# amolchanov86/gym_art

Hardware: AMD Instinct MI355X
Metric: env-steps/sec (whole node) at N=2^20 Hummingbird; achieved HBM GB/s (higher is better)
Workload: dtype f64

## Files before the change

gym_art_amd/csrc/gaq.hip:

```cpp
#include "gaq_host.hpp"

#define GAQ_X(FEAT) extern template __global__ GAQ_STEP_SIG(FEAT)
GAQ_STEP_ALL(GAQ_X)
#undef GAQ_X
#define GAQ_X(FEAT) extern template __global__ GAQ_ROLL_SIG(FEAT)
GAQ_ROLL_ALL(GAQ_X)
#undef GAQ_X

namespace {

using namespace gaqk;

__global__ __launch_bounds__(kBlock) void episode_kernel(int64_t n, const float* __restrict__ reward,
                                                          const uint8_t* __restrict__ done, float* __restrict__ ep_ret,
                                                          uint32_t* __restrict__ ep_len, double* __restrict__ acc) {
  const int64_t i = (int64_t)blockIdx.x * kBlock + threadIdx.x;
  float ret = 0.0f; uint32_t len = 0; bool fin = false;
  if (i < n) {
    ret = ep_ret[i] + reward[i];
    len = ep_len[i] + 1u;
    fin = done[i] != 0;
    ep_ret[i] = fin ? 0.0f : ret;
    ep_len[i] = fin ? 0u : len;
  }
// ... 141 lines not shown
      float* row = reinterpret_cast<float*>(rows) + lane * D;
      if (alias && !hi_out) {
#pragma unroll
        for (int k = 0; k < 18; ++k) row[k] = hi18[k];
      } else {
        const float* sz = p.sense_in;
        const int64_t n = p.n;
        double t2w = 0.0, t2t = 0.0;
        if (cfg.obs_flags & (gaq::OBS_APPEND_T2W | gaq::OBS_APPEND_T2T)) {
          double th[4], tq0 = um.torque_max[0], im = um.inv_mass;
#pragma unroll
          for (int j = 0; j < 4; ++j) th[j] = um.thrust_max[j];
          if (p.par) {
#pragma unroll
            for (int j = 0; j < 4; ++j) th[j] = t.ld64(p.par, kPar, PP_THRUST_MAX + j);
            tq0 = t.ld64(p.par, kPar, PP_TORQUE_MAX); im = t.ld64(p.par, kPar, PP_INV_MASS);
          }
          t2w = (((th[0] + th[1]) + th[2]) + th[3]) * im / 9.81; t2t = tq0 / th[0];
        }
        gaq::pack_obs<double, gaq::F_GENERIC | gaq::F_DIAG>(s, cfg, acc, hist, [&](int k, float v, int) { row[k] = v; },
                                            cfg.env_offset + (uint64_t)i, cfg.step_index, 1, WaveSwarm{lane, cfg.swarm.agents},
                                            [&](int c, int slot, int j) { return sz ? sz[((int64_t)(c * 12 + slot) * 3 + j) * n + i] : 0.0f; }, t2w, t2t);
        if (cfg.gyro_bias && (!do_reset || mask == nullptr || mask[i])) {
#pragma unroll
          for (int j = 0; j < 3; ++j) t.st32(p.gyro, j, s.gyro_bias[j]);
        }
      }
    }
  }
  if (obs) {
    wave_lds_fence();
    flush_obs(obs, p.n, D, tile, rows, lane);
  }
}

__global__ __launch_bounds__(kBlock) void export_kernel(DevPtrs p, int alias, double* __restrict__ out, float* __restrict__ aux_out = nullptr) {
  const int64_t i = (int64_t)blockIdx.x * kBlock + threadIdx.x;
  if (i >= p.n) return;
  if (aux_out) {
    for (int k = 0; k < gaq::AUX_WORDS; ++k) aux_out[i * gaq::AUX_WORDS + k] = p.aux[i * gaq::AUX_WORDS + k];
  }
  const int64_t n = p.n;
  const int64_t tile = i / kTile;
  const int lane = (int)(i % kTile);
  auto grp = [&](const float* a, int plane) { return (double)a[tile * (4 * kTile) + plane * kTile + lane]; };
  for (int k = 0; k < 3; ++k) out[(34 + k) * n + i] = grp(p.goal, k);
  if (alias) {
    for (int k = 0; k < 18; ++k)
      out[(int64_t)k * n + i] = lo_decode(alias, p.obs_in, p.lo, i, k) + (k < 3 ? grp(p.goal, k) : 0.0);
  } else {
    for (int k = 0; k < kCorePlanes; ++k) out[(int64_t)k * n + i] = p.core[tile * (kCorePlanes * kTile) + k * kTile + lane];
  }
  for (int j = 0; j < 4; ++j) {
    out[(18 + j) * n + i] = p.lag[tile * (kLagPlanes * kTile) + j * kTile + lane];
    out[(22 + j) * n + i] = grp(p.cmds, j);
    out[(26 + j) * n + i] = grp(p.ou, j);
    out[(30 + j) * n + i] = grp(p.actp, j);
  }
  const uint32_t c = p.ctr[i];
  out[37 * n + i] = (double)(c & 0xFFFFu);
  out[38 * n + i] = (double)(c >> 16);
  for (int k = 0; k < 3; ++k) out[(39 + k) * n + i] = grp(p.gyro, k);
}

thread_local std::string g_err;

int svd_period_of(double dt) {
  double t = 0.0; int k = 0;
  while (!(t > 0.5)) { t += dt; ++k; if (k > 1000000) break; }
  return k;
}

}

int fail(int code, const std::string& msg) { g_err = msg; return code; }
int env_override(const char* name) { const char* v = getenv(name); return v ? (v[0] == '1' ? 1 : 0) : -1; }
LaunchRecord& launch_record() { static LaunchRecord r; return r; }

namespace {

Overrides read_overrides() {
  return {env_override("GAQ_FORCE_GENERIC") == 1, env_override("GAQ_NO_AUXP") == 1, env_override("GAQ_PREDRAW"), env_override("GAQ_NT")};
}

struct Layout { bool alias, pack, shadow, fp32; };
struct Selection { uint32_t variant; bool generic; int lds_per_wave; };
struct ParamFlags { bool lag, drag; };
struct Plan { Layout layout; Selection sel; };

bool step_instantiated(uint32_t f) {
  switch (f) {
#define GAQ_X(FEAT) case (FEAT):
    GAQ_STEP_ALL(GAQ_X)
#undef GAQ_X
      return true;
    default: return false;
  }
}
bool roll_instantiated(uint32_t f) {
  switch (f) {
#define GAQ_X(FEAT) case (FEAT):
    GAQ_ROLL_ALL(GAQ_X)
#undef GAQ_X
      return true;
    default: return false;
  }
}

const void* step_kernel_ptr(uint32_t f) {
  switch (f) {
#define GAQ_X(FEAT) case (FEAT): return (const void*)&step_kernel<(FEAT)>;
    GAQ_STEP_ALL(GAQ_X)
#undef GAQ_X
    default: return nullptr;
  }
}
uint32_t rollout_variant_of(uint32_t variant, const Layout& L, bool generic) {
  const uint32_t base = variant & ~(gaq::F_PREDRAW | gaq::F_NT | gaq::F_ROWS | gaq::F_CTR);
  if (!L.alias || L.pack || generic || (variant & gaq::F_MELL)) return 0xFFFFFFFFu;
  if ((base >= 16u && base <= 23u) || (variant >= 48u && variant <= 55u)) return base;
  return 0xFFFFFFFFu;
}

uint32_t rows_twin_of(uint32_t variant) { return step_instantiated(variant | gaq::F_ROWS) ? (variant | gaq::F_ROWS) : 0xFFFFFFFFu; }
uint32_t ctr_twin_of(uint32_t variant) { return step_instantiated(variant | gaq::F_CTR) ? (variant | gaq::F_CTR) : 0xFFFFFFFFu; }

int observation_dim(const gaq_config* cfg) {
  int D = (cfg->obs_flags & GAQ_OBS_QUAT) ? 13 : 18;
  if (cfg->obs_flags & GAQ_OBS_APPEND_T2W) D += 1;
  if (cfg->obs_flags & GAQ_OBS_APPEND_T2T) D += 1;
  if (cfg->obs_flags & GAQ_OBS_APPEND_H) D += 1;
  if (cfg->obs_flags & GAQ_OBS_APPEND_ACC) D += 3;
  if (cfg->obs_flags & GAQ_OBS_APPEND_ACT) D += 4;
  if (cfg->swarm.agents > 1) D += 6 * (cfg->swarm.agents - 1);
  return D;
}

int fill_step_cfg(const gaq_config* cfg, StepCfg& sc, int& obs_dim) {
  if (cfg->struct_size != sizeof(gaq_config) || cfg->abi_version != GAQ_ABI_VERSION)
    return fail(GAQ_ERR_INVALID, "gaq_config size/version mismatch (header vs library)");
  if (cfg->num_envs <= 0) return fail(GAQ_ERR_INVALID, "num_envs must be positive");
  if (cfg->num_envs > (int64_t)1 << 27) return fail(GAQ_ERR_INVALID, "num_envs above 2^27 per handle is not supported");
  if (!(cfg->sim_freq > 0) || cfg->sim_steps <= 0) return fail(GAQ_ERR_INVALID, "sim_freq and sim_steps must be positive");
  if (cfg->sim_steps > 64)
    return fail(GAQ_ERR_INVALID, "sim_steps above 64 is not supported (random-stream ids of the sub-steps)");
  if (cfg->ep_len < 0 || cfg->ep_len >= 0xFFFF) return fail(GAQ_ERR_INVALID, "ep_len must be in [0, 65534]");
  if (cfg->control < 0 || cfg->control > 2) return fail(GAQ_ERR_INVALID, "unknown control mode");
  if (cfg->noise < 0 || cfg->noise > 2) return fail(GAQ_ERR_INVALID, "unknown noise mode");
  if (cfg->reward_mode < 0 || cfg->reward_mode > 1) return fail(GAQ_ERR_INVALID, "unknown reward mode");
  if (cfg->obs_flags & ~127) return fail(GAQ_ERR_INVALID, "unknown obs flags");
  if ((cfg->obs_flags & GAQ_OBS_QUAT) && cfg->swarm.agents > 1) return fail(GAQ_ERR_INVALID, "the quaternion observation is not available for swarms");
  if (cfg->swarm.agents > 1) {
    const int a = cfg->swarm.agents;
    if (a > 16 || (a & (a - 1)) != 0) return fail(GAQ_ERR_INVALID, "swarm.agents must be a power of two <= 16");
    if (cfg->num_envs % a != 0 || cfg->env_id_offset % a != 0)
      return fail(GAQ_ERR_INVALID, "num_envs and env_id_offset must be multiples of swarm.agents (whole worlds per handle)");
    if (!(cfg->swarm.prox_dist > 0.0f) || !(cfg->swarm.collision_dist >= 0.0f) || !(cfg->swarm.goal_radius >= 0.0f))
      return fail(GAQ_ERR_INVALID, "swarm distances must be positive");
  }
  const double dt = 1.0 / cfg->sim_freq;
  const int period = svd_period_of(dt);
  if (period >= 0xFFFF) return fail(GAQ_ERR_INVALID, "sim_freq too high for the 16-bit SVD counter");
  if (cfg->sim_freq < 50.0) return fail(GAQ_ERR_INVALID, "sim_freq below 50 Hz is outside the rotation series' range");
  const int D = observation_dim(cfg);
  obs_dim = D;
  std::memset(&sc, 0, sizeof(sc));
// ... 429 lines not shown
  if (e->stage_bytes > ((size_t)1 << 20)) return GAQ_OK;
  const bool zc = env_override("GAQ_ZERO_COPY") != 0;
  HIP_TRY(hipHostMalloc((void**)&e->stage_pin, e->stage_bytes, zc ? hipHostMallocMapped : hipHostMallocDefault));
  if (zc) e->stage_map = device_view(e->stage_pin);
  return GAQ_OK;
}

struct Transport {
  char* io;
  char* home;
  bool copy_in;
  bool own_obs;
};
Transport transport_of(const gaq_env* e) {
  const bool mapped = e->stage_map != nullptr;
  const bool own_obs = e->alias && !e->pack && !(mapped && e->shadow);
  return {mapped ? e->stage_map : e->stage_dev, e->stage_pin, !mapped, own_obs};
}

}

int sync_handle(gaq_env* e) {
  HIP_TRY(hipStreamSynchronize(e->stream));
  if (e->user_stream_used) HIP_TRY(hipStreamSynchronize(e->user_stream));
  return GAQ_OK;
}

int check_overrun(gaq_env* e) {
  if (!e->d.rz_overrun) return GAQ_OK;
  uint32_t o = 0;
  HIP_TRY(hipMemcpy(&o, e->d.rz_overrun, sizeof(uint32_t), hipMemcpyDeviceToHost));
  if (o) return fail(GAQ_ERR_STATE, "internal: an env was re-randomised before its staged parameter planes were refilled");
  return GAQ_OK;
}

extern "C" {

int gaq_abi_version(void) { return GAQ_ABI_VERSION; }
const char* gaq_last_error(void) { return g_err.c_str(); }

int gaq_num_devices(void) {
  int n = 0;
  if (hipGetDeviceCount(&n) != hipSuccess) return 0;
  return n;
}

int gaq_create(const gaq_config* cfg, gaq_env** out) {
  if (!cfg || !out) return fail(GAQ_ERR_INVALID, "null argument");
  StepCfg sc0;
  int D = 18;
  if (int rc = fill_step_cfg(cfg, sc0, D)) return rc;
  if (!cfg->per_env_params && check_model(cfg->model) != GAQ_OK) return GAQ_ERR_INVALID;
  int ndev = gaq_num_devices();
  if (ndev <= 0) return fail(GAQ_ERR_DEVICE, "no HIP device visible: libgaq has no CPU fallback");
  if (cfg->device < 0 || cfg->device >= ndev) return fail(GAQ_ERR_INVALID, "device ordinal out of range");
  HIP_TRY(hipSetDevice(cfg->device));
  hipDeviceProp_t prop;
  HIP_TRY(hipGetDeviceProperties(&prop, cfg->device));

  gaq_env* e = new (std::nothrow) gaq_env();
  if (!e) return fail(GAQ_ERR_DEVICE, "out of host memory");
  e->cfg = *cfg;
  e->obs_dim = D;
  e->num_cus = prop.multiProcessorCount > 0 ? prop.multiProcessorCount : 256;
  StepCfg& sc = e->sc;
  sc = sc0;
  const double dt = sc.dt;

  if (!cfg->per_env_params) {
    derive_model(cfg->model, dt, e->um);
    e->um.jinv = nullptr;
    if (cfg->control == GAQ_CTRL_MELLINGER && !inverse_jacobian(cfg->model, sc.jinv)) {
      delete e;
      return fail(GAQ_ERR_INVALID, "singular quadrotor jacobian");
    }
  } else {
    std::memset(&e->um, 0, sizeof(e->um));
  }
  { const ParamFlags f = start_flags(*cfg, e->um); e->any_lag = f.lag; e->any_drag = f.drag; }
  { const char* nf = getenv("GAQ_NO_FUSED"); if (nf && nf[0] == '1') e->fused_rollout = false; }
  e->ov = read_overrides();
  e->lomix = cfg->per_env_params != 0 || e->any_lag;
  { const char* ca = getenv("GAQ_CHECK_ALIAS"); e->check_alias = ca && ca[0] == '1'; }
  {
    const char* ab = getenv("GAQ_ABLATE");
    sc.ablate = ab ? atoi(ab) : 0;
    if (sc.ablate != 0 && !kDiagBuild) {
      delete e;
      return fail(GAQ_ERR_INVALID, "GAQ_ABLATE is set but this libgaq is not a measurement build (make EXTRA=-DGAQ_DIAG_BUILD OUT=...): "
                                   "the ablations skip parts of the step and give wrong physics; unset the variable");
    }
    if (sc.ablate != 0) fprintf(stderr, "libgaq: GAQ_ABLATE=%d in a measurement build -- results are WRONG by construction, only timings mean anything\n", sc.ablate);
  }
  refresh_feature_flags(e);
  if (e->fp32 && !e->alias) {
    delete e;
    return fail(GAQ_ERR_INVALID, "fp32_state needs the specialised kernels (18-word world-frame obs, RawControl, default reward terms)");
  }
  if (!step_instantiated((uint32_t)e->variant)) {
    delete e;
    return fail(GAQ_ERR_STATE, "internal: no kernel instantiation for this feature mask");
  }

  DevPtrs& d = e->d;
  std::memset(&d, 0, sizeof(d));
  d.n = cfg->num_envs;
  d.ntiles = (cfg->num_envs + kTile - 1) / kTile;
  {
    uint64_t waves;
    counter_plan(d.ntiles, waves, d.ctr_shift, d.ctr_inc0);
  }
  const size_t nt = (size_t)d.ntiles;
  hipError_t he = hipSuccess;
  auto alloc0 = [&](void** p, size_t bytes) {
    if (he != hipSuccess) return;
    he = hipMalloc(p, bytes);
    if (he == hipSuccess) he = hipMemset(*p, 0, bytes);
  };
  if (e->alias) {
    if (!e->fp32) alloc0((void**)&d.lo, nt * (e->lomix ? (size_t)kMixRowsBytes : (size_t)kLoRowsBytes));
    alloc0((void**)&e->own_obs, nt * kRowsBytes);
  } else {
    alloc0((void**)&d.core, nt * kCoreBytes);
  }
  alloc0((void**)&d.lag, nt * kLagBytes);
  alloc0((void**)&d.ou, nt * kGrpBytes);
  alloc0((void**)&d.cmds, nt * kGrpBytes);
  alloc0((void**)&d.actp, nt * kGrpBytes);
  alloc0((void**)&d.goal, nt * kGrpBytes);
  alloc0((void**)&d.gyro, nt * kGrpBytes);
  alloc0((void**)&e->step_ctr_mem, sizeof(uint64_t) * kCtrSlots * kCtrStride);
  alloc0((void**)&e->alias_sum_dev, sizeof(uint64_t));
  alloc0((void**)&d.ctr, nt * kTile * sizeof(uint32_t));
  alloc0((void**)&d.done_count, sizeof(uint32_t) * 2);
  alloc0((void**)&d.nan_count, sizeof(uint32_t));
  if (cfg->compact_done) alloc0((void**)&d.done_list, nt * kTile * sizeof(uint32_t));
  if (cfg->aux_outputs) alloc0((void**)&d.aux, nt * kTile * gaq::AUX_WORDS * sizeof(float));
  if (cfg->per_env_params) {
    double* par = nullptr;
    double* jinv_dev = nullptr;
    alloc0((void**)&par, nt * kParBytes);
    if (cfg->control == GAQ_CTRL_MELLINGER) alloc0((void**)&jinv_dev, nt * kTile * 16 * sizeof(double));
    d.par = par;
    d.jinv = jinv_dev;
    alloc0((void**)&d.traj, 4 * nt * kTile * sizeof(uint32_t));
    d.rcount = d.traj ? d.traj + nt * kTile : nullptr;
    d.rz_flag = d.traj ? d.traj + 2 * nt * kTile : nullptr;
    e->host_par.assign(nt * kPar * kTile, 1.0);
    for (size_t t = 0; t < nt; ++t)
      for (int pl : {(int)PP_VEL_DAMP, (int)PP_DAMP_Q, (int)PP_C_DRAG, (int)PP_C_ROLL, (int)PP_COMX, (int)PP_COMY, (int)PP_OU_SIGMA})
        std::fill_n(e->host_par.begin() + (t * kPar + pl) * kTile, kTile, 0.0);
    e->pflags.assign((size_t)cfg->num_envs, 0);
  }
  if (he == hipSuccess) he = hipStreamCreateWithFlags(&e->stream, hipStreamNonBlocking);
  if (he == hipSuccess) he = hipEventCreate(&e->ev0);
  if (he == hipSuccess) he = hipEventCreate(&e->ev1);
  if (he != hipSuccess) {
    std::string msg = std::string("device allocation failed: ") + hipGetErrorString(he);
    gaq_destroy(e);
    return fail(GAQ_ERR_DEVICE, msg);
  }
  auto init_state = [&]() -> int {
    std::vector<float> goal(nt * 4 * kTile, 0.0f);
    for (int64_t i = 0; i < d.ntiles * kTile; ++i) {
      goal[tidx(i, 4, 2)] = 2.0f;
      if (sc.swarm.agents > 1) {
// ... 517 lines not shown
```

gym_art_amd/csrc/gaq_kernels.hpp:

```cpp
#pragma once

#include <hip/hip_runtime.h>

#include <cstddef>
#include <cstdint>

#include "../../include/gaq.h"
#include "quad_core.hpp"
#include "quad_params_dev.hpp"

namespace gaqk {

#ifndef GAQ_LD_AUX
#define GAQ_LD_AUX 0
#endif
#ifndef GAQ_ST_AUX
#define GAQ_ST_AUX 0
#endif
#ifndef GAQ_ACT_AUX
#define GAQ_ACT_AUX 0
#endif
template <uint32_t F> constexpr int kLdAux = (F & gaq::F_NT) ? 2 : GAQ_LD_AUX;
template <uint32_t F> constexpr int kStAux = (F & gaq::F_NT) ? 2 : GAQ_ST_AUX;
#ifndef GAQ_COPY_AUX
#define GAQ_COPY_AUX 2
#endif
template <uint32_t F> constexpr int kCopyAux = (F & gaq::F_NT) ? 2 : GAQ_COPY_AUX;
#ifdef GAQ_DIAG_BUILD
constexpr bool kDiagBuild = true;
#else
constexpr bool kDiagBuild = false;
#endif
__host__ __device__ __forceinline__ bool ablated(const gaq::StepCfg& cfg, int bit) { return kDiagBuild && (cfg.ablate & bit) != 0; }
constexpr int kBlock = 256;
constexpr int kTile = 64;
constexpr int kCorePlanes = 18;
constexpr int kLagPlanes = 4;
constexpr int kCoreBytes = kCorePlanes * kTile * 8;
constexpr int kLagBytes = kLagPlanes * kTile * 8;
constexpr int kGrpBytes = 4 * kTile * 4;
constexpr int kRowBytes = 18 * 4;
constexpr int kRowsBytes = kTile * kRowBytes;
constexpr int kRowsLds = 5 * 1024;
constexpr int kLoRowBytes = 18 * 2;
constexpr int kLoRowsBytes = kTile * kLoRowBytes;
constexpr int kLoRowsLds = 3 * 1024;
constexpr int kMixRowWords = 11;
constexpr int kMixRowBytes = kMixRowWords * 4;
constexpr int kMixRowsBytes = kTile * kMixRowBytes;
template <uint32_t F> constexpr bool kLoMix = (F & (gaq::F_PER_ENV | gaq::F_LAG)) != 0;
constexpr int kPar = 45;
constexpr int kParBytes = kPar * kTile * 8;
constexpr int kHotPlanes = 19;
constexpr int kParNextSkew = 544;
enum ParPlane { PP_MASS = 0, PP_INV_MASS = 1, PP_INERTIA = 2, PP_INV_INERTIA = 5, PP_THRUST_MAX = 8, PP_TORQUE_MAX = 12,
                PP_PROP_X = 16, PP_PROP_Y = 20, PP_PROP_Z = 24, PP_TAU_UP = 28, PP_TAU_DOWN = 29, PP_LINEARITY = 30,
                PP_ARM = 31, PP_VEL_DAMP = 32, PP_DAMP_Q = 33, PP_C_DRAG = 34, PP_C_ROLL = 35, PP_OU_SIGMA = 36,
                PP_T2T = 37, PP_MX = 38, PP_MY = 39, PP_COMX = 40, PP_COMY = 41, PP_COMPACT_OK = 42,
                PP_T_UP = 43, PP_T_DOWN = 44 };

struct DevPtrs {
  double* core;
  void* lo;
  const float* obs_in;
  float* obs_copy;
  float* hi_final;
  double* lag;
  float* ou;
  float* cmds;
  float* actp;
  float* goal;
  float* gyro;
  uint32_t* ctr;
  const double* par;
  const double* jinv;
  const float* noise_in;
  const float* sense_in;
  float* aux;
  uint32_t* done_list;
  uint32_t* done_count;
  uint32_t* nan_count;
  float* term_obs;
  float* ep_ret;
  uint32_t* ep_len;
  double* ep_acc;
  uint64_t* step_ctr;
  uint32_t ctr_shift;
  uint32_t ctr_inc0;
  float* rows_out;
  uint32_t* rcount;
  uint32_t* traj;
  double* par_next;
  uint32_t* rz_flag;
  uint32_t* rz_overrun;
  int32_t rz_every;
  int64_t n, ntiles;
};

using gaq::EnvState;
using gaq::Model;
using gaq::StepCfg;

template <uint32_t F> struct RealOf { using type = double; };
// ... 477 lines not shown
__device__ __forceinline__ void flush_packed_rows(float* rows_out, int64_t n, int W, int64_t tile, char* lds, uint32_t lane) {
  const int64_t first = tile * kTile;
  const int64_t live = (n - first) < kTile ? (n - first) : kTile;
  const uint32_t bytes = (uint32_t)live * W * 4u;
  auto r = __builtin_amdgcn_make_buffer_rsrc(rows_out + first * W, 0, (int)bytes, 0x00020000);
  const int pieces = (kTile * W * 4 + 1023) / 1024;
  for (int k = 0; k < pieces; ++k) {
    const uint32_t off = k * 1024 + lane * 16u;
    if (off < (uint32_t)(kTile * W * 4)) {
      const u32x4 v = *reinterpret_cast<const u32x4*>(lds + off);
      __builtin_amdgcn_raw_buffer_store_b128(v, r, off, 0, AUX);
    }
  }
}

__device__ __forceinline__ void store_aux(const DevPtrs& p, int64_t i, const gaq::StepOut& out) {
  if (!p.aux) return;
  float* ax = p.aux + i * gaq::AUX_WORDS;
#pragma unroll
  for (int j = 0; j < 3; ++j) { ax[gaq::AUX_ACC + j] = out.acc_meter[j]; ax[gaq::AUX_OMEGA_DOT + j] = out.omega_dot[j]; ax[gaq::AUX_TORQUE + j] = out.torque[j]; }
#pragma unroll
  for (int j = 0; j < 4; ++j) { ax[gaq::AUX_CTRL + j] = out.ctrl[j]; ax[gaq::AUX_CMDS + j] = out.cmds[j]; }
}

struct KernArgsMirror { DevPtrs p; StepCfg cfg; Model<double> um; };
static_assert(offsetof(KernArgsMirror, um) == sizeof(DevPtrs) + sizeof(StepCfg) && sizeof(DevPtrs) % 8 == 0 && sizeof(StepCfg) % 8 == 0,
              "kernel-argument layout of step_kernel's first three arguments");
typedef __attribute__((address_space(4))) const char karg_char;
__device__ __forceinline__ karg_char* kernarg_model_ptr() {
#if defined(__HIP_DEVICE_COMPILE__)
  return (karg_char*)__builtin_amdgcn_kernarg_segment_ptr() + offsetof(KernArgsMirror, um);
#else
  return nullptr;
#endif
}

constexpr int kArgLines = 18;
static_assert((kArgLines - 1) * 64 + 4 <= (int)sizeof(KernArgsMirror) && kArgLines * 64 >= (int)sizeof(KernArgsMirror),
              "kernarg_warm covers the by-value arguments and reads nothing behind them");
__device__ __forceinline__ uint32_t kernarg_warm() {
  uint32_t token = 0;
#if defined(__HIP_DEVICE_COMPILE__)
  asm("s_load_dword %0, %1, 0x0\n\ts_load_dword %0, %1, 0x40\n\ts_load_dword %0, %1, 0x80\n\ts_load_dword %0, %1, 0xc0\n\t"
      "s_load_dword %0, %1, 0x100\n\ts_load_dword %0, %1, 0x140\n\ts_load_dword %0, %1, 0x180\n\ts_load_dword %0, %1, 0x1c0\n\t"
      "s_load_dword %0, %1, 0x200\n\ts_load_dword %0, %1, 0x240\n\ts_load_dword %0, %1, 0x280\n\ts_load_dword %0, %1, 0x2c0\n\t"
      "s_load_dword %0, %1, 0x300\n\ts_load_dword %0, %1, 0x340\n\ts_load_dword %0, %1, 0x380\n\ts_load_dword %0, %1, 0x3c0\n\t"
      "s_load_dword %0, %1, 0x400\n\ts_load_dword %0, %1, 0x440"
      : "=&s"(token)
      : "s"((karg_char*)__builtin_amdgcn_kernarg_segment_ptr()));
  __builtin_amdgcn_sched_barrier(0);
#endif
  return token;
}
template <uint32_t F> constexpr int kArgPrologue = 2;
#define GAQ_ARG_PROLOGUE(FEAT, FORM) template <> inline constexpr int kArgPrologue<(FEAT)> = (FORM);
GAQ_ARG_PROLOGUE(66578u, 1) GAQ_ARG_PROLOGUE(66577u, 1) GAQ_ARG_PROLOGUE(68627u, 1) GAQ_ARG_PROLOGUE(19477u, 1) GAQ_ARG_PROLOGUE(197653u, 1)
GAQ_ARG_PROLOGUE(197654u, 1) GAQ_ARG_PROLOGUE(197655u, 1) GAQ_ARG_PROLOGUE(199699u, 1)
#undef GAQ_ARG_PROLOGUE
template <uint32_t F, int FORM = 2, typename C, typename A>
__device__ __forceinline__ C kernarg_batch(uint32_t token, C carry, const DevPtrs& p, A actions, int lds_per_wave) {
  if constexpr (FORM == 1) {
    asm("s_waitcnt lgkmcnt(0)" : "+s"(carry) : "s"(token), "s"(p.ntiles), "s"(p.n), "s"(p.step_ctr));
    return carry;
  }
  if constexpr ((F & gaq::F_GENERIC) == 0) {
    if constexpr ((F & gaq::F_LAG) != 0) asm("" : "+s"(carry) : "s"(p.lag), "s"(p.cmds));
    if constexpr ((F & gaq::F_NOISE) != 0) asm("" : "+s"(carry) : "s"(p.ou));
  }
  if constexpr ((F & gaq::F_ALIAS) != 0) {
    asm("s_waitcnt lgkmcnt(0)" : "+s"(carry) : "s"(token), "s"(p.ntiles), "s"(p.n), "s"(p.step_ctr), "s"(p.ctr_shift), "s"(p.obs_in), "s"(p.lo),
        "s"(p.ctr), "s"(actions), "s"(lds_per_wave));
  } else {
    asm("s_waitcnt lgkmcnt(0)" : "+s"(carry) : "s"(token), "s"(p.ntiles), "s"(p.n), "s"(p.step_ctr), "s"(p.ctr_shift), "s"(p.core), "s"(p.ctr),
        "s"(actions), "s"(lds_per_wave));
  }
  return carry;
}

template <uint32_t F> constexpr int kStepMinWaves = 1;
#ifndef GAQ_NO_FLOORS
template <> inline constexpr int kStepMinWaves<214036u> = 3;
template <> inline constexpr int kStepMinWaves<82962u> = 3;
#endif
template <uint32_t F>
__global__ __launch_bounds__(kBlock) __attribute__((amdgpu_waves_per_eu(kStepMinWaves<F>))) void step_kernel(DevPtrs p, StepCfg cfg, Model<double> um,
                                                       const float* __restrict__ actions, float* obs,
                                                       float* __restrict__ reward, uint8_t* __restrict__ done,
                                                       int lds_per_wave) {
  constexpr bool G = (F & gaq::F_GENERIC) != 0;
  constexpr bool A = (F & gaq::F_ALIAS) != 0;
  static_assert(!(G && A), "obs/state aliasing exists in the specialised kernels only");
  extern __shared__ __attribute__((aligned(16))) char smem[];
  int wave_ = __builtin_amdgcn_readfirstlane(threadIdx.x >> 6);
  if constexpr (kArgPrologue<F> != 0) wave_ = kernarg_batch<F, kArgPrologue<F>>(kernarg_warm(), wave_, p, actions, lds_per_wave);
  const int wave = wave_;
  const uint32_t lane = threadIdx.x & 63u;
  const int64_t tile = (int64_t)blockIdx.x * (kBlock / kTile) + wave;
  if constexpr ((F & gaq::F_CTR) != 0) {
    if (tile >= p.ntiles) {
      (void)step_counter_checkin(p, step_counter_read(p, lane), lane);
      return;
    }
  } else {
    if (p.step_ctr) cfg.step_index = *p.step_ctr >> p.ctr_shift;
    if (tile >= p.ntiles) return;
  }
  char* buf = smem + wave * lds_per_wave;
  const int64_t i = tile * kTile + lane;
  const bool live = i < p.n;
  const int D = cfg.obs_dim;

  stage_in<F>(p, cfg, tile, buf, lane);
  if constexpr (kArgPrologue<F> == 2) __builtin_amdgcn_sched_barrier(0);
  using T = Real<F>;
  Model<T> m;
  if constexpr (!gaq::kModelMem<F>) load_model<F>(p, cfg, tile, lane, um, m);
  const Model<T>* mp = &m;
  if constexpr (gaq::kModelMem<F>) mp = (const Model<T>*)kernarg_model_ptr();
  float4 a4;
  uint32_t cw;
  {
    auto ra = __builtin_amdgcn_make_buffer_rsrc(const_cast<float*>(actions), 0, (int)(p.n * 16), 0x00020000);
    const u32x4 v = __builtin_amdgcn_raw_buffer_load_b128(ra, (uint32_t)i * 16u, 0, (F & gaq::F_NT) ? 2 : GAQ_ACT_AUX);
    a4 = __builtin_bit_cast(float4, v);
    auto rc = __builtin_amdgcn_make_buffer_rsrc(p.ctr, 0, (int)(p.ntiles * kTile * 4), 0x00020000);
    cw = __builtin_amdgcn_raw_buffer_load_b32(rc, (uint32_t)i * 4u, 0, (F & gaq::F_NT) ? 2 : GAQ_ACT_AUX);
  }
  if constexpr ((F & gaq::F_CTR) != 0) cfg.step_index = step_counter_checkin(p, step_counter_read(p, lane), lane);
  float pre0[4] = {0.0f, 0.0f, 0.0f, 0.0f}, pre1[4] = {0.0f, 0.0f, 0.0f, 0.0f};
  if constexpr ((F & gaq::F_PREDRAW) != 0) {
    const gaq::Philox r0(cfg.seed, cfg.env_offset + (uint64_t)i, cfg.step_index, gaq::RNG_OU0);
    gaq::normals4(r0, pre0);
    if (cfg.sim_steps > 1) { const gaq::Philox r1(cfg.seed, cfg.env_offset + (uint64_t)i, cfg.step_index, gaq::RNG_OU0 + 1u); gaq::normals4(r1, pre1); }
  }
  if constexpr ((F & gaq::F_PREDRAW) != 0) {
    asm volatile("" :: "v"(pre0[0]), "v"(pre0[1]), "v"(pre0[2]), "v"(pre0[3]), "v"(pre1[0]), "v"(pre1[1]), "v"(pre1[2]), "v"(pre1[3]));
  }
  wait_dma();
  EnvState<T> s;
  read_image<F>(cfg, buf, lane, s);
  s.tick = cw & 0xFFFFu;
  s.svd_ctr = cw >> 16;
  wave_lds_fence();

  const float act[4] = {a4.x, a4.y, a4.z, a4.w};
  gaq::StepOut out;
  out.reward = 0.0f; out.done = 0; out.crashed = 0;
  constexpr int kObWords = (F & gaq::F_AUXP) ? 28 : 26;
  float ob[kObWords];
#pragma unroll
  for (int k = 0; k < kObWords; ++k) ob[k] = 0.0f;
  char* rows = buf;
  float* term_row = p.term_obs ? p.term_obs + i * D : nullptr;
#ifndef GAQ_PACK_ROWS_LDS
#define GAQ_PACK_ROWS_LDS 0
#endif
  constexpr bool kObsRowsInLds = G || (F & gaq::F_SWARM) != 0 || (F & gaq::F_AUXP) != 0 ||
                                 (GAQ_PACK_ROWS_LDS && (F & gaq::F_PACK) != 0 && (F & gaq::F_ALIAS) != 0);
  constexpr bool kAuxRowsInLds = gaq::kAuxIsRow<F>;
  const int aux_off = (kTile * D * 4 + 15) & ~15;
  if (live && !ablated(cfg, 1)) {
    if constexpr ((F & gaq::F_SWARM) != 0) {
      float* row = reinterpret_cast<float*>(rows) + lane * D;
      gaq::env_step<T, F>(s, *mp, cfg, act, cfg.env_offset + (uint64_t)i, [&](int, int) { return 0.0f; }, out,
                          [&](int k, float v, int) { row[k] = v; }, term_row, WaveSwarm{lane, cfg.swarm.agents});
    } else if constexpr (G) {
      const float* nz = p.noise_in;
      const int64_t n = p.n;
      float* row = reinterpret_cast<float*>(rows) + lane * D;
      if constexpr (kAuxRowsInLds) out.aux_row = reinterpret_cast<float*>(rows + aux_off) + lane * gaq::AUX_WORDS;
      const float* sz = p.sense_in;
      gaq::env_step<T, F>(s, *mp, cfg, act, cfg.env_offset + (uint64_t)i,
                               [&](int k, int c) { return nz[((int64_t)k * 4 + c) * n + i]; }, out,
                               [&](int k, float v, int) { row[k] = v; }, term_row, WaveSwarm{lane, cfg.swarm.agents},
                               [&](int c, int slot, int j) { return sz ? sz[((int64_t)(c * 12 + slot) * 3 + j) * n + i] : 0.0f; });
      if constexpr (gaq::kAux<F> && !kAuxRowsInLds) store_aux(p, i, out);
    } else if constexpr (gaq::kHeadsAreObs<F>) {
      gaq::env_step<T, F>(s, *mp, cfg, act, cfg.env_offset + (uint64_t)i, [&](int k, int c) { return k == 0 ? pre0[c] : pre1[c]; }, out,
                          [&](int, float, int) {}, term_row);
    } else if constexpr (kObsRowsInLds) {
      float* row = reinterpret_cast<float*>(rows) + lane * D;
      if constexpr (kAuxRowsInLds) out.aux_row = reinterpret_cast<float*>(rows + aux_off) + lane * gaq::AUX_WORDS;
      gaq::env_step<T, F>(s, *mp, cfg, act, cfg.env_offset + (uint64_t)i, [&](int, int) { return 0.0f; }, out,
                          [&](int k, float v, int) { row[k] = v; }, term_row);
      if constexpr (gaq::kAux<F> && !kAuxRowsInLds) store_aux(p, i, out);
    } else {
      gaq::env_step<T, F>(s, *mp, cfg, act, cfg.env_offset + (uint64_t)i, [&](int, int) { return 0.0f; }, out,
                          [&](int k, float v, int slot) { if (slot < 0) ob[k] = v; else ob[18 + slot] = v; }, term_row);
      if constexpr (gaq::kAux<F>) store_aux(p, i, out);
    }
  }
  bool promote = false;
  if constexpr ((F & gaq::F_RZ) != 0) {
    if (p.rz_every > 0 && live && out.done && !ablated(cfg, 4)) {
      auto rt = __builtin_amdgcn_make_buffer_rsrc(p.traj, 0, (int)(p.ntiles * (3 * kTile * 4)), 0x00020000);
      const int third = (int)(p.ntiles * (kTile * 4));
      bool due = true;
      if (p.rz_every > 1) {
        const uint32_t tr = __builtin_amdgcn_raw_buffer_load_b32(rt, (uint32_t)i * 4u, 0, 0) + 1u;
        __builtin_amdgcn_raw_buffer_store_b32(tr, rt, (uint32_t)i * 4u, 0, 0);
        due = ((tr + 1u) % (uint32_t)p.rz_every) == 0u;
      }
      if (due) {
        promote = true;
        (void)__builtin_amdgcn_raw_ptr_buffer_atomic_add_i32(1, rt, (uint32_t)i * 4u, third, 0);
        (void)__builtin_amdgcn_raw_ptr_buffer_atomic_add_i32(1, rt, (uint32_t)i * 4u, 2 * third, 0);
        s.svd_ctr = 0;
#pragma unroll
        for (int j = 0; j < 4; ++j) s.ou[j] = 0.0f;
      }
    }
  }
  if constexpr (kObsRowsInLds) {
    wave_lds_fence();
    if constexpr (A) flush_obs(p.obs_copy, p.n, D, tile, rows, lane);
    else flush_obs(obs, p.n, D, tile, rows, lane);
    if constexpr (kAuxRowsInLds) { if (p.aux) flush_obs(p.aux, p.n, gaq::AUX_WORDS, tile, rows + aux_off, lane); }
    wave_lds_fence();
  }
  write_image<F>(cfg, buf, lane, s);
  wave_lds_fence();
  stage_out<F>(p, cfg, tile, buf, lane, obs);
  {
    auto rc = __builtin_amdgcn_make_buffer_rsrc(p.ctr, 0, (int)(p.ntiles * kTile * 4), 0x00020000);
    __builtin_amdgcn_raw_buffer_store_b32((s.tick & 0xFFFFu) | (s.svd_ctr << 16), rc, (uint32_t)i * 4u, 0, kStAux<F>);
  }
  if (live) {
    reward[i] = out.reward;
    done[i] = out.done;
    if (!isfinite(out.reward)) atomicAdd(p.nan_count, 1u);
  }
  if constexpr (!gaq::kHeadsAreObs<F> && !kObsRowsInLds) {
    float* obs_rows_out = obs;
    if constexpr (A) obs_rows_out = p.obs_copy;
    wave_lds_fence();
    float* row = reinterpret_cast<float*>(rows) + lane * D;
    if (D == 18) {
#pragma unroll
      for (int k = 0; k < 18; k += 2) *reinterpret_cast<float2*>(row + k) = make_float2(ob[k], ob[k + 1]);
    } else {
      int k = 18;
      bool quat = false;
      if constexpr ((F & gaq::F_AUXP) != 0) quat = (cfg.obs_flags & gaq::OBS_QUAT) != 0;
      if (quat) {
#pragma unroll
        for (int j = 0; j < 13; ++j) row[j] = ob[j];
        k = 13;
      } else {
#pragma unroll
        for (int j = 0; j < 18; ++j) row[j] = ob[j];
      }
      if (cfg.obs_flags & gaq::OBS_APPEND_H) row[k++] = ob[18];
      if (cfg.obs_flags & gaq::OBS_APPEND_ACC) { row[k] = ob[19]; row[k + 1] = ob[20]; row[k + 2] = ob[21]; k += 3; }
      if (cfg.obs_flags & gaq::OBS_APPEND_ACT) { row[k] = ob[22]; row[k + 1] = ob[23]; row[k + 2] = ob[24]; row[k + 3] = ob[25]; k += 4; }
      if constexpr ((F & gaq::F_AUXP) != 0) {
        if (cfg.obs_flags & gaq::OBS_APPEND_T2W) row[k++] = ob[26];
        if (cfg.obs_flags & gaq::OBS_APPEND_T2T) row[k++] = ob[27];
      }
    }
    wave_lds_fence();
    flush_obs(obs_rows_out, p.n, D, tile, rows, lane);
  }

  if constexpr ((F & gaq::F_ROWS) != 0) {
    static_assert(gaq::kHeadsAreObs<F> && (F & gaq::F_FP32) == 0, "fused packed rows: alias kernels whose observation is the heads");
    float hv[18];
    const float2* h = reinterpret_cast<const float2*>(buf + lane * kRowBytes);
#pragma unroll
    for (int k = 0; k < 9; ++k) { const float2 a = h[k]; hv[2 * k] = a.x; hv[2 * k + 1] = a.y; }
    wave_lds_fence();
    float* row = reinterpret_cast<float*>(buf) + lane * 20;
#pragma unroll
    for (int k = 0; k < 18; k += 2) *reinterpret_cast<float2*>(row + k) = make_float2(hv[k], hv[k + 1]);
    *reinterpret_cast<float2*>(row + 18) = make_float2(out.reward, (float)out.done);
    wave_lds_fence();
    flush_packed_rows<kStAux<F>>(p.rows_out, p.n, 20, tile, buf, lane);
  }

  if constexpr ((F & gaq::F_RZ) != 0) {
    unsigned long long pm = __ballot(promote);
    if (pm && !ablated(cfg, 2)) {
      double* cur = const_cast<double*>(p.par) + tile * (int64_t)(kPar * kTile);
      const double* rows = p.par + p.ntiles * (int64_t)(kPar * kTile) + kParNextSkew + tile * (int64_t)(kPar * kTile);
      const bool hot_only = cfg.compact_params != 0 && cfg.zero_damp != 0 && (F & gaq::F_FP32) == 0;
      const int pl = hot_only ? (int)lane + ((int)lane < 4 ? 1 : (int)lane < 9 ? 4 : (int)lane < 13 ? 19 : 23) : (int)lane;
      static_assert(PP_INV_MASS == 1 && PP_INERTIA == 2 && PP_THRUST_MAX == 8 && PP_TORQUE_MAX == 12 && PP_TAU_UP == 28 && PP_TAU_DOWN == 29 &&
                    PP_LINEARITY == 30 && PP_ARM == 31 && PP_OU_SIGMA == 36 && PP_T2T == 37 && PP_COMY == 41, "hot planes of a promotion");
      const bool mine = hot_only ? (int)lane < kHotPlanes : (int)lane < kPar;
      while (pm) {
        const int L = __ffsll((long long)pm) - 1;
        pm &= pm - 1ull;
        if (mine) {
          const double v = rows[L * kPar + pl];
          if (pl == PP_OU_SIGMA) reinterpret_cast<float*>(cur + PP_OU_SIGMA * kTile)[L] = (float)v;
          else cur[pl * kTile + L] = v;
        }
      }
    }
  }
  if (p.done_list) {
    const bool is_done = live && out.done;
    uint32_t* cnt = p.done_count + (cfg.step_index & 1);
    if (i == 0) p.done_count[(cfg.step_index + 1) & 1] = 0;
    const unsigned long long mask = __ballot(is_done);
    if (mask) {
      const int leader = __ffsll((long long)mask) - 1;
      uint32_t base = 0;
      if ((int)lane == leader) base = atomicAdd(cnt, (uint32_t)__popcll(mask));
      base = __shfl(base, leader);
      if (is_done) p.done_list[base + __popcll(mask & ((1ull << lane) - 1ull))] = (uint32_t)i;
    }
  }
// ... 323 lines not shown
```

gym_art_amd/csrc/quad_core.hpp:

```cpp
#pragma once

#include <stdint.h>
#include <math.h>

#if defined(__HIPCC__)
#define GAQ_HD __host__ __device__ __forceinline__
#else
#define GAQ_HD inline
#endif

#if defined(__HIP_DEVICE_COMPILE__)
#define GAQ_SINF(x) __sinf(x)
#define GAQ_COSF(x) __cosf(x)
#define GAQ_LOGF(x) __logf(x)
#ifndef GAQ_REWARD_SQRT_FAST
#define GAQ_REWARD_SQRT_FAST 1
#endif
#if GAQ_REWARD_SQRT_FAST
#define GAQ_SQRTF_OUT(x) __builtin_amdgcn_sqrtf(x)
#else
#define GAQ_SQRTF_OUT(x) sqrtf(x)
#endif
#else
#define GAQ_SINF(x) sinf(x)
// ... 37 lines not shown
template <uint32_t F> GAQ_HD void model_fence() {
#if defined(__HIP_DEVICE_COMPILE__)
  if constexpr (kModelMem<F>) asm volatile("" ::: "memory");
#endif
}
template <uint32_t F> constexpr bool kSwarm = (F & F_GENERIC) != 0 || (F & F_SWARM) != 0;
template <uint32_t F> constexpr bool kHeadsAreObs = (F & F_ALIAS) != 0 && (F & F_PACK) == 0;
template <uint32_t F> constexpr bool kDiag = (F & F_GENERIC) != 0 && (F & F_LITE) == 0 && (F & F_DIAG) != 0;
template <uint32_t F> constexpr bool kAuxIsRow =
#if defined(__HIP_DEVICE_COMPILE__)
    (F & F_AUXP) != 0 || ((F & F_GENERIC) != 0 && (F & F_DIAG) != 0);
#else
    false;
#endif
template <uint32_t F> constexpr bool kAux = kDiag<F> || ((F & F_GENERIC) != 0 && (F & F_LITE) != 0 && (F & F_DIAG) != 0) || (F & F_AUXP) != 0;

enum ControlMode { CTRL_RAW_ZERO_MIDDLE = 0, CTRL_RAW = 1, CTRL_MELLINGER = 2 };
enum NoiseMode { NOISE_OFF = 0, NOISE_PHILOX = 1, NOISE_INPUT = 2 };
enum RewardMode { REW_QUADROTOR = 0, REW_MULTI_LOG = 1 };
enum ObsFlags { OBS_BODY_FRAME = 1, OBS_APPEND_H = 2, OBS_APPEND_ACC = 4, OBS_APPEND_ACT = 8,
                OBS_QUAT = 16 , OBS_APPEND_T2W = 32, OBS_APPEND_T2T = 64  };

struct RewCoeff {
  float pos, effort, crash, orient, yaw, rot, attitude, spin, action_change, vel;
  float pos_offset, pos_log_weight, pos_linear_weight;
};

struct SenseNoise {
  int32_t enabled;
  float pos_norm_std, pos_unif_range, vel_norm_std, vel_unif_range, quat_norm_std, quat_unif_range;
  float gyro_noise_density, acc_static_noise_std, acc_dynamic_noise_ratio;
  float gyro_norm_std, gyro_random_walk, gyro_bias_correlation_time;
};

struct SwarmCfg {
  int32_t agents;
  float goal_radius;
  float collision_dist;
  float prox_dist;
  float w_collision, w_prox;
  int32_t response;
};

template <typename T>
struct Model {
  T mass, inv_mass;
  T inertia[3], inv_inertia[3];
  T thrust_max[4], torque_max[4];
  T prop_x[4], prop_y[4], prop_z[4];
  T tau_up, tau_down;
  T linearity, arm, vel_damp, damp_omega_q, c_drag, c_roll;
  float ou_sigma;
  const double* jinv;
};

struct StepCfg {
  double dt;
  double gravity;
  double room_lo[3], room_hi[3];
  double goal_default[3];
  double init_box;
  int32_t sim_steps, ep_len, svd_period;
  int32_t control, noise, reward_mode, obs_flags, obs_dim;
  int32_t motor_lag;
  int32_t drag;
  int32_t need_act_prev;
  int32_t per_env_goal;
  int32_t resample_goal;
  int32_t excite;
  int32_t auto_reset, init_random_state;
  int32_t use_acos;
  RewCoeff rew;
  SenseNoise sense;
  SwarmCfg swarm;
  int32_t compact_params;
  int32_t zero_damp;
  int32_t action_f32;
  int32_t sense_input;
  int32_t aux;
  int32_t ablate;
  int32_t gyro_bias;
  float gyro_pi, gyro_sigma, gyro_pi_step, gyro_sigma_step;
  float t2w_std, t2w_min, t2w_max, t2t_std, t2t_min, t2t_max;
  double jinv[16];
  uint64_t seed, step_index, env_offset;
};

template <uint32_t F> GAQ_HD bool has_lag(const StepCfg& c) { if constexpr ((F & F_GENERIC) != 0) return c.motor_lag != 0; else return (F & F_LAG) != 0; }
template <uint32_t F> GAQ_HD int noise_mode(const StepCfg& c) {
  if constexpr ((F & F_GENERIC) != 0 && (F & F_LITE) != 0) return c.noise == NOISE_PHILOX ? NOISE_PHILOX : NOISE_OFF;
  else if constexpr ((F & F_GENERIC) != 0) return c.noise;
  else return (F & F_NOISE) ? NOISE_PHILOX : NOISE_OFF;
}
template <uint32_t F> GAQ_HD bool has_act_prev(const StepCfg& c) { if constexpr (kHeadsAreObs<F>) return false; else return c.need_act_prev != 0; }
template <uint32_t F> GAQ_HD bool has_env_goal(const StepCfg& c) {
  if constexpr ((F & F_GENERIC) != 0 || (F & F_ENVX) != 0) return c.per_env_goal != 0; else return (F & F_SWARM) != 0;
}
template <uint32_t F> GAQ_HD int swarm_agents(const StepCfg& c) { if constexpr (kSwarm<F>) return c.swarm.agents; else return 0; }
template <uint32_t F> constexpr bool kGyroBias = ((F & F_GENERIC) != 0 && (F & F_LITE) == 0) || (F & F_BIAS) != 0;
template <uint32_t F> GAQ_HD bool has_gyro_bias(const StepCfg& c) { if constexpr (kGyroBias<F>) return c.gyro_bias != 0; else return false; }

template <typename T>
struct EnvState {
  T pos[3], vel[3], rot[9], omega[3];
  T rot_damp[4];
  float cmds_damp[4];
  float ou[4];
  float act_prev[4];
  T goal[3];
  float gyro_bias[3];
  uint32_t tick, svd_ctr;
};

struct StepOut {
  float reward;
  uint8_t done, crashed;
  float acc_meter[3];
  float omega_dot[3], torque[3], ctrl[4], cmds[4];
  float* aux_row = nullptr;
};
enum { AUX_ACC = 0, AUX_OMEGA_DOT = 3, AUX_TORQUE = 6, AUX_CTRL = 9, AUX_CMDS = 13, AUX_WORDS = 17 };

GAQ_HD double clampv(double x, double lo, double hi) { return fmin(fmax(x, lo), hi); }
GAQ_HD float clampv(float x, float lo, float hi) { return fminf(fmaxf(x, lo), hi); }
GAQ_HD double sqrt_t(double x) { return sqrt(x); }
GAQ_HD float sqrt_t(float x) { return sqrtf(x); }

GAQ_HD double split_decode(float hi, uint32_t q) {
  const uint64_t b = __builtin_bit_cast(uint64_t, (double)hi) | ((uint64_t)(q & 0xFFFFu) << 13);
  return __builtin_bit_cast(double, b);
}
GAQ_HD float split_hi(double v) {
  const float h = (float)v;
  uint32_t hb = __builtin_bit_cast(uint32_t, h);
  if (fabs((double)h) > fabs(v)) hb -= 1u;
  return __builtin_bit_cast(float, hb);
}
GAQ_HD double split_decode32(float hi, uint32_t q) {
  return __builtin_bit_cast(double, __builtin_bit_cast(uint64_t, (double)hi) | (uint64_t)(q & 0x1FFFFFFFu));
}
GAQ_HD uint32_t split_lo32(double v) {
  return (uint32_t)__builtin_bit_cast(uint64_t, v) & 0x1FFFFFFFu;
}
GAQ_HD uint32_t split_lo(double v) {
  return (uint32_t)(__builtin_bit_cast(uint64_t, v) >> 13) & 0xFFFFu;
}

template <typename T>
GAQ_HD void sinc_cosc(T q, T& A, T& B) {
  const float qf = (float)q;
  float ta = -8.2206352466243297e-18f;
  ta = fmaf(ta, qf, 2.8114572543455206e-15f);
  ta = fmaf(ta, qf, -7.6471637318198164e-13f);
  ta = fmaf(ta, qf, 1.6059043836821613e-10f);
  ta = fmaf(ta, qf, -2.5052108385441720e-08f);
  ta = fmaf(ta, qf, 2.7557319223985893e-06f);
  float tb = -4.1103176233121648e-19f;
  tb = fmaf(tb, qf, 1.5619206968586225e-16f);
  tb = fmaf(tb, qf, -4.7794773323873853e-14f);
  tb = fmaf(tb, qf, 1.1470745597729725e-11f);
  tb = fmaf(tb, qf, -2.0876756987868100e-09f);
  tb = fmaf(tb, qf, 2.7557319223985888e-07f);
  A = T(1.0) + q * (T(-1.0 / 6) + q * (T(1.0 / 120) + q * (T(-1.0 / 5040) + q * T(ta))));
  B = T(0.5) + q * (T(-1.0 / 24) + q * (T(1.0 / 720) + q * (T(-1.0 / 40320) + q * T(tb))));
}

// ... 836 lines not shown
```

Baseline: 21.88 billion.

## Alternate block-to-tile sweep direction per step to reuse cache across launches

On odd steps the step kernel remaps each block index to a mirrored position within its XCD's round-robin group, so tiles touched last in one launch are processed first in the next and may still sit in L2/MALL. This targets HBM traffic for the state read back each step. It also adds optional nontemporal stores for reward/done and a separate action-load cache-policy macro, both off by default. The remap costs a few scalar ops per block and is disabled for two specific variants; step_index is now read before the tile is computed.

```diff
diff --git a/gym_art_amd/csrc/gaq.hip b/gym_art_amd/csrc/gaq.hip
--- a/gym_art_amd/csrc/gaq.hip
+++ b/gym_art_amd/csrc/gaq.hip
@@ -247,6 +247,7 @@
 Overrides read_overrides() {
   return {env_override("GAQ_FORCE_GENERIC") == 1, env_override("GAQ_NO_AUXP") == 1, env_override("GAQ_PREDRAW"), env_override("GAQ_NT")};
 }
+constexpr int kSweepDefault = 1;
 
 struct Layout { bool alias, pack, shadow, fp32; };
 struct Selection { uint32_t variant; bool generic; int lds_per_wave; };
@@ -842,6 +843,7 @@
   e->ov = read_overrides();
   e->lomix = cfg->per_env_params != 0 || e->any_lag;
   { const char* ca = getenv("GAQ_CHECK_ALIAS"); e->check_alias = ca && ca[0] == '1'; }
+  { const int sw = env_override("GAQ_SWEEP"); sc.sweep = sw < 0 ? kSweepDefault : sw; }
   {
     const char* ab = getenv("GAQ_ABLATE");
     sc.ablate = ab ? atoi(ab) : 0;
diff --git a/gym_art_amd/csrc/gaq_kernels.hpp b/gym_art_amd/csrc/gaq_kernels.hpp
--- a/gym_art_amd/csrc/gaq_kernels.hpp
+++ b/gym_art_amd/csrc/gaq_kernels.hpp
@@ -19,6 +19,12 @@
 #endif
 #ifndef GAQ_ACT_AUX
 #define GAQ_ACT_AUX 0
+#endif
+#ifndef GAQ_ACTION_AUX
+#define GAQ_ACTION_AUX GAQ_ACT_AUX
+#endif
+#ifndef GAQ_OUT_NT
+#define GAQ_OUT_NT 0
 #endif
 template <uint32_t F> constexpr int kLdAux = (F & gaq::F_NT) ? 2 : GAQ_LD_AUX;
 template <uint32_t F> constexpr int kStAux = (F & gaq::F_NT) ? 2 : GAQ_ST_AUX;
@@ -662,6 +668,10 @@
 template <> inline constexpr int kStepMinWaves<214036u> = 3;
 template <> inline constexpr int kStepMinWaves<82962u> = 3;
 #endif
+constexpr uint32_t kXcds = 8;
+template <uint32_t F> constexpr bool kSweeps = true;
+template <> inline constexpr bool kSweeps<17428u> = false;
+template <> inline constexpr bool kSweeps<2569u> = false;
 template <uint32_t F>
 __global__ __launch_bounds__(kBlock) __attribute__((amdgpu_waves_per_eu(kStepMinWaves<F>))) void step_kernel(DevPtrs p, StepCfg cfg, Model<double> um,
                                                        const float* __restrict__ actions, float* obs,
@@ -675,14 +685,23 @@
   if constexpr (kArgPrologue<F> != 0) wave_ = kernarg_batch<F, kArgPrologue<F>>(kernarg_warm(), wave_, p, actions, lds_per_wave);
   const int wave = wave_;
   const uint32_t lane = threadIdx.x & 63u;
-  const int64_t tile = (int64_t)blockIdx.x * (kBlock / kTile) + wave;
+  uint32_t block = blockIdx.x;
+  if constexpr ((F & gaq::F_CTR) == 0) {
+    if (p.step_ctr) cfg.step_index = *p.step_ctr >> p.ctr_shift;
+    if constexpr (kSweeps<F>) {
+      const uint32_t nblocks = (uint32_t)((p.ntiles + (kBlock / kTile - 1)) / (kBlock / kTile));
+      const uint32_t xcd = block % kXcds, members = (nblocks - xcd + (kXcds - 1u)) / kXcds;
+      const uint32_t mirrored = xcd + (members - 1u - block / kXcds) * kXcds;
+      block = ((uint32_t)cfg.sweep & (uint32_t)cfg.step_index & 1u) != 0 ? mirrored : block;
+    }
+  }
+  const int64_t tile = (int64_t)block * (kBlock / kTile) + wave;
   if constexpr ((F & gaq::F_CTR) != 0) {
     if (tile >= p.ntiles) {
       (void)step_counter_checkin(p, step_counter_read(p, lane), lane);
       return;
     }
   } else {
-    if (p.step_ctr) cfg.step_index = *p.step_ctr >> p.ctr_shift;
     if (tile >= p.ntiles) return;
   }
   char* buf = smem + wave * lds_per_wave;
@@ -701,7 +720,7 @@
   uint32_t cw;
   {
     auto ra = __builtin_amdgcn_make_buffer_rsrc(const_cast<float*>(actions), 0, (int)(p.n * 16), 0x00020000);
-    const u32x4 v = __builtin_amdgcn_raw_buffer_load_b128(ra, (uint32_t)i * 16u, 0, (F & gaq::F_NT) ? 2 : GAQ_ACT_AUX);
+    const u32x4 v = __builtin_amdgcn_raw_buffer_load_b128(ra, (uint32_t)i * 16u, 0, (F & gaq::F_NT) ? 2 : GAQ_ACTION_AUX);
     a4 = __builtin_bit_cast(float4, v);
     auto rc = __builtin_amdgcn_make_buffer_rsrc(p.ctr, 0, (int)(p.ntiles * kTile * 4), 0x00020000);
     cw = __builtin_amdgcn_raw_buffer_load_b32(rc, (uint32_t)i * 4u, 0, (F & gaq::F_NT) ? 2 : GAQ_ACT_AUX);
@@ -806,8 +825,8 @@
     __builtin_amdgcn_raw_buffer_store_b32((s.tick & 0xFFFFu) | (s.svd_ctr << 16), rc, (uint32_t)i * 4u, 0, kStAux<F>);
   }
   if (live) {
-    reward[i] = out.reward;
-    done[i] = out.done;
+    if constexpr (GAQ_OUT_NT != 0) { __builtin_nontemporal_store(out.reward, &reward[i]); __builtin_nontemporal_store(out.done, &done[i]); }
+    else { reward[i] = out.reward; done[i] = out.done; }
     if (!isfinite(out.reward)) atomicAdd(p.nan_count, 1u);
   }
   if constexpr (!gaq::kHeadsAreObs<F> && !kObsRowsInLds) {
diff --git a/gym_art_amd/csrc/quad_core.hpp b/gym_art_amd/csrc/quad_core.hpp
--- a/gym_art_amd/csrc/quad_core.hpp
+++ b/gym_art_amd/csrc/quad_core.hpp
@@ -143,6 +143,7 @@
   int32_t gyro_bias;
   float gyro_pi, gyro_sigma, gyro_pi_step, gyro_sigma_step;
   float t2w_std, t2w_min, t2w_max, t2t_std, t2t_min, t2t_max;
+  int32_t sweep;
   double jinv[16];
   uint64_t seed, step_index, env_offset;
 };
```

New measurement: 22.18 billion, median of 6. +1.4%, better.
